# akio-tomiya/LatticeQCD.jl

Measured on AMD Instinct MI355X. Metric: CG iters/sec (D^+D) & Dslash GFLOP/s, 32^3x64 SU(3) Wilson fp64, higher is better.
Workload: dtype f64; 1 GPU; configs[3]: 32x32x32x64 Wilson D^+D CG (fixed-length window), fp64; dslash_variant=1, xcd_remap=2, xcd_nsub=16, xcd_ysplit=4, cg_fused=3, gauge_recon=12, gauge_recon_active=1, comm_backend=none, comm_requested=auto

## Files before the change

latticeqcd.jl_amd/csrc/capi.hip:

```cpp
#include "lqcd_internal.h"

#include <algorithm>
#include <cstdio>
#include <cstdlib>
#include <cstring>
#include <mutex>

namespace lqcd {

static thread_local std::string g_err;
static std::mutex g_live_mu;
static std::vector<const lqcd_ctx_s*> g_live;
bool ctx_is_live(const lqcd_ctx_s* c) {
    std::lock_guard<std::mutex> lk(g_live_mu);
    for (const lqcd_ctx_s* p : g_live)
        if (p == c) return true;
    return false;
}
static void ctx_set_live(const lqcd_ctx_s* c, bool live) {
    std::lock_guard<std::mutex> lk(g_live_mu);
    for (size_t i = 0; i < g_live.size(); i++)
        if (g_live[i] == c) { g_live.erase(g_live.begin() + i); break; }
    if (live) g_live.push_back(c);
}
// ... 283 lines not shown
    if (!strcmp(key, "clover_hop_s")) return &c->tun.clover_hop_s;
    if (!strcmp(key, "mixed_lean_residual")) return &c->tun.mixed_lean_residual;
    if (!strcmp(key, "mixed_xfuse")) return &c->tun.mixed_xfuse;
    if (!strcmp(key, "mixed_defer_x")) return &c->tun.mixed_defer_x;
    if (!strcmp(key, "pair32_active")) return &c->tun.pair32_active;
    if (!strcmp(key, "stag_both")) return &c->tun.stag_both;
    if (!strcmp(key, "clover_fused")) return &c->tun.clover_fused;
    if (!strcmp(key, "clover_transport")) return &c->tun.clover_transport;
    if (!strcmp(key, "halo_stream_mode")) return &c->tun.halo_stream_mode;
    if (!strcmp(key, "cg_skip_done")) return &c->tun.cg_skip_done;
    if (!strcmp(key, "cg_small")) return &c->tun.cg_small;
    if (!strcmp(key, "cg_tgauge")) return &c->tun.cg_tgauge;
    if (!strcmp(key, "tgauge_active")) return &c->tun.tgauge_active;
    if (!strcmp(key, "cg_sweep_alt")) return &c->tun.cg_sweep_alt;
    if (!strcmp(key, "cg_sweep_alt_active")) return &c->tun.cg_sweep_alt_active;
    if (!strcmp(key, "dslash_sweep")) return &c->tun.dslash_sweep;
    if (!strcmp(key, "sweep_rev_active")) return &c->tun.sweep_rev_active;
    if (!strcmp(key, "dslash_xshare")) return &c->tun.dslash_xshare;
    if (!strcmp(key, "xshare_active")) return &c->tun.xshare_active;
    if (!strcmp(key, "dslash_yshare")) return &c->tun.dslash_yshare;
    if (!strcmp(key, "yshare_active")) return &c->tun.yshare_active;
    if (!strcmp(key, "nt_centre")) return &c->tun.nt_centre;
    if (!strcmp(key, "cg_persist")) return &c->tun.cg_persist;
    if (!strcmp(key, "md_remap")) return &c->tun.md_remap;
    if (!strcmp(key, "staple_recon")) return &c->tun.staple_recon;
    if (!strcmp(key, "staple_tile")) return &c->tun.staple_tile;
    if (!strcmp(key, "md_reunitarize")) return &c->tun.md_reunitarize;
    if (!strcmp(key, "nt_blas")) return &c->tun.nt_blas;
    if (!strcmp(key, "cg_fold_scalars")) return &c->tun.cg_fold_scalars;
    if (!strcmp(key, "halo_fuse")) return &c->tun.halo_fuse;
// ... 45 lines not shown
extern "C" int lqcd_ctx_set_param(lqcd_ctx_t c, const char* key, int value) {
    ARGCHK(c && key, "lqcd_ctx_set_param: null");
    if (!strcmp(key, "adopt_thread")) {
        {
            std::lock_guard<std::mutex> lk(g_live_mu);
            c->home_thread = std::this_thread::get_id();
        }
        return ctx_drain_parked(c);
    }
    int* p = param_ptr(c, key);
    ARGCHK(p, std::string("lqcd_ctx_set_param: unknown key ") + key);
    if (!strcmp(key, "dslash_block")) ARGCHK(value == 64 || value == 128 || value == 256, "dslash_block must be 64, 128 or 256");
    if (!strcmp(key, "halo_stream_mode")) ARGCHK(value >= -1 && value <= 4, "halo_stream_mode must be -1 (timed once) or 0..4");
    if (!strcmp(key, "cg_rring")) ARGCHK(value == 0 || value == 2 || value == 4 || value == 8, "cg_rring must be 0 (off), 2, 4 or 8 (it divides the 8 iterations of a captured burst)");
    if (!strcmp(key, "cg_rring_mult")) ARGCHK((value == 1 || value == 2 || value == 4) && std::max(c->tun.cg_rring, 1) * value <= RRING_MAX, "cg_rring_mult must be 1, 2 or 4 with cg_rring x cg_rring_mult <= 32");
    if (!strcmp(key, "scratch_max")) ARGCHK(value >= 0, "scratch_max: 0 (no limit) or the number of work fields the scratch pool may hold");
    if (!strcmp(key, "bicg_fused")) ARGCHK(value != 3, "bicg_fused must be 0, 1, 2 or 4 (3, the grid-barrier form, was measured slower and removed)");
    if (!strcmp(key, "halo_inject_us")) ARGCHK(value >= 0 && value <= 100000, "halo_inject_us: 0..100000");
    if ((!strcmp(key, "lazy_links") || !strcmp(key, "lazy_merge")) && !value) LQCHK(links_flush_of(c));
    if (*p != value) LQCHK(links_flush_of(c));
    *p = value;
    if (!strcmp(key, "cg_rring_mult")) c->tun.cg_rring_mult_set = 1;
    return LQCD_OK;
}
extern "C" int lqcd_ctx_get_param(lqcd_ctx_t c, const char* key, int* value) {
    ARGCHK(c && key && value, "lqcd_ctx_get_param: null");
    if (!strcmp(key, "dw_active")) { *value = c->tun.dw_active; return LQCD_OK; }
    if (!strcmp(key, "adopt_thread")) {
        std::lock_guard<std::mutex> lk(g_live_mu);
        *value = std::this_thread::get_id() == c->home_thread ? 1 : 0;
        return LQCD_OK;
    }
    if (!strcmp(key, "parked_fields")) {
        std::lock_guard<std::mutex> lk(g_live_mu);
        *value = (int)c->parked_gauges.size();
        return LQCD_OK;
    }
// ... 100 lines not shown
```

latticeqcd.jl_amd/csrc/cg.hip:

```cpp
#include "ops_internal.h"
#include "stencil_common.h"

#include <algorithm>
#include <cmath>

namespace lqcd {


__global__ void cg_scalar_alpha(double* s) {
    if (s[S_DONE] != 0.0) { s[S_XDONE] = 1.0; return; }
    s[S_ALPHA] = s[S_RR] / s[S_PQ];
}
__global__ void cg_scalar_beta(double* s) {
    if (s[S_DONE] != 0.0) return;
    const double rrn = s[S_RRNEW];
    s[S_BETA] = rrn / s[S_RR];
    s[S_RR] = rrn;
    s[S_ITERS] += 1.0;
    if (rrn < s[S_EPS]) s[S_DONE] = 1.0;
}

__global__ __launch_bounds__(UB) void cg_update_xr(const double* __restrict__ s, double2* __restrict__ x, double2* __restrict__ r,
                                                    const double2* __restrict__ p, const double2* __restrict__ q, size_t n,
                                                    double* partial) {
// ... 441 lines not shown
    StencilCall s1;
    if (m == 0) {
        LQCHK(cg_batch_launch(c, x, w, 0));
        apply_bc(c, op->bc);
        LQCHK(make_full_call(op, w.tmp, w.p, 0, s1));
        s1.skip_flag = c->tun.cg_skip_done ? c->d_scal : nullptr;
    } else {
        apply_bc(c, op->bc);
        LQCHK(make_full_call(op, w.tmp, rk, 0, s1));
        s1.upd_scal = c->d_scal;
        s1.upd[0] = spinor_block(w.tmp, 0);
        s1.upd[1] = spinor_block(w.tmp, 1);
        s1.upd_rec = 1;
    }
    s1.gauge12t = gt;
    s1.norm_partial = c->d_partial;
    LQCHK(stencil_apply(c, s1));
    LQCHK(reduce_to_slot(c, nbs, 1, S_PQ, true, m == 0 ? 9 : 7));
    apply_bc(c, op->bc);
    StencilCall s2;
    LQCHK(make_full_call(op, rn, w.tmp, 1, s2));
    s2.gauge12t = gt;
    s2.sweep_rev = w.sweep_alt ? 1 : 0;
    s2.norm_partial = c->d_partial;
    s2.upd_scal = c->d_scal;
    for (int q = 0; q < 2; q++) { s2.upd[q] = spinor_block(rn, q); s2.upd_src[q] = spinor_block(rk, q); }
    LQCHK(stencil_apply(c, s2));
    LQCHK(reduce_to_slot(c, nbs, 1, S_RRNEW, true, 8));
    w.k++;
    return LQCD_OK;
}
static int cg_rring_wanted(lqcd_op_s* op, const CgWork& w) {
    lqcd_ctx_s* c = op->ctx;
    const int K = c->tun.cg_rring;
    if (c->tun.cg_fused < 3 || !(K == 2 || K == 4 || K == 8)) return 0;
    if (op->kind != LQCD_WILSON || op->r != 1.0 || op->csw != 0.0 || any_partitioned(c) || c->has_comm || !c->local_peers.empty()) return 0;
    if (!stencil_sdir_applies(c, op->kind, op->r, op_fused_clover(op))) return 0;
    StencilCall s;
// ... 77 lines not shown
    const int nbs = stencil_num_partials(c, op->kind, op->r, 2, 0, op_fused_clover(op));
    const bool defer = w.form == CgForm::DeferX;
    const bool ringed = defer && w.ring > 2;
    lqcd_spinor_s* pk = ringed ? w.buf(w.k % w.ring) : (defer && (w.k & 1)) ? w.q : w.p;
    lqcd_spinor_s* po = ringed ? w.buf((w.k + 1) % w.ring) : (defer && (w.k & 1)) ? w.p : w.q;
    const bool fold = c->has_comm && defer && c->tun.cg_fold_scalars;
    const bool part = any_partitioned(c) && c->has_comm && c->local_peers.empty();
    const bool folded = part && halo_fold_applies(c, op->kind, op->r, 2, 0, op_fused_clover(op));
    const bool fr = part && (c->tun.halo_fuse & 1) && !folded;
    const bool fp = part && defer && (c->tun.halo_fuse & 2) && op->kind == LQCD_WILSON && op->r == 1.0;
    {
        apply_bc(c, op->bc);
        StencilCall s1;
        LQCHK(make_full_call(op, w.tmp, pk, 0, s1));
        s1.gauge12t = gt;
        s1.norm_partial = c->d_partial;
        s1.skip_flag = c->tun.cg_skip_done ? c->d_scal : nullptr;
        if (fr) s1.red_slot = S_PQ;
        if (fp) { s1.pack_next = 1; s1.prepacked = (w.p_packed && w.pack_epoch == c->halo_epoch) ? 1 : 0; s1.defer_pack = folded ? 1 : 0; }
        LQCHK(stencil_apply(c, s1));
    }
    LQCHK(fr ? reduce_tail(c, 1, S_PQ, fold ? 0 : 1) : reduce_pack_to_slot(c, nbs, S_PQ, fold ? 0 : 1));
    apply_bc(c, op->bc);
    StencilCall s2;
    LQCHK(make_full_call(op, po, w.tmp, 1, s2));
    s2.gauge12t = gt;
    s2.sweep_rev = w.sweep_alt ? 1 : 0;
    s2.norm_partial = c->d_partial;
    if (fold) s2.scal_w = c->d_scal;
    s2.upd_scal = c->d_scal;
    s2.upd[0] = spinor_block(w.r, 0);
    s2.upd[1] = spinor_block(w.r, 1);
    if (fr) s2.red_slot = S_RRNEW;
    if (fp) s2.prepacked = 1;
    LQCHK(stencil_apply(c, s2));
    LQCHK(fr ? reduce_tail(c, 1, S_RRNEW, fold ? 0 : 2) : reduce_to_slot(c, nbs, 1, S_RRNEW, true, fold ? 0 : 2));
    const int nbu = stream_grid(c, n);
    HArgs h = HArgs();
    int npx = 0, npack = 0;
    if (fp) {
        int nt = 0;
        for (int mu = 0; mu < 4; mu++)
// ... 55 lines not shown
    if (!ok) for (lqcd_spinor_s*& f : w.more) { if (f) scratch_put(f); f = nullptr; }
    return ok;
}
static CgForm cg_choose_form(lqcd_op_s* op, CgWork& w) {
    lqcd_ctx_s* c = op->ctx;
    const int fused = c->tun.cg_fused;
    if (fused >= 2 && c->tun.cg_small && cg_small_ok(op, stencil_num_partials(c, op->kind, op->r, 2, 0, op_fused_clover(op)))) return CgForm::Small;
    if (const int K = cg_rring_wanted(op, w)) {
        for (int M = cg_rring_mult_wanted(op, K); M >= 1; M >>= 1)
            if (cg_more_get(c, w, K * M)) { w.rring = K * M; w.rring_k = K; return CgForm::RRing; }
    }
    if (fused >= 2 && c->tun.cg_defer_x) return CgForm::DeferX;
    return fused >= 2 ? CgForm::Fused : fused ? CgForm::NormFused : CgForm::Reference;
}

int cg_setup(lqcd_op_s* op, lqcd_spinor_s* x, lqcd_spinor_s* b, CgWork& w, double eps, double* rr0) {
    lqcd_ctx_s* c = op->ctx;
    const size_t n = x->elems;
    LQCHK(halo_schedule_settle(op));
    w.tgauge = cg_tgauge_wanted(op);
    c->tun.tgauge_active = w.tgauge ? 1 : 0;
    w.links_t = w.tgauge ? op->gauge->data12t : nullptr;
    w.gfix = w.tgauge ? op->gauge->gfix : nullptr;
    w.gauge_version = op->gauge->version;
    if (w.tgauge) LQCHK(spinor_gauge_rotate(c, w.gfix, x->data, x->data, 0));
    LQCHK(op_apply_async(op, w.tmp, x, 0, nullptr, nullptr, w.links_t));
    LQCHK(op_apply_async(op, w.q, w.tmp, 1, nullptr, nullptr, w.links_t));
    if (w.tgauge) LQCHK(spinor_gauge_rotate(c, w.gfix, w.r->data, b->data, 0));
    else HIPCHK(hipMemcpyAsync(w.r->data, b->data, n * sizeof(double2), hipMemcpyDeviceToDevice, c->stream));
    LQCHK(blas_axpy(c, -1.0, 0.0, w.q->data, w.r->data, n));
    HIPCHK(hipMemcpyAsync(w.p->data, w.r->data, n * sizeof(double2), hipMemcpyDeviceToDevice, c->stream));
    LQCHK(blas_norm2(c, w.r->data, n, rr0, true));
    double init[12] = {*rr0, 0, 0, 0, 0, 0, eps, 0, 0, 0, 0, 0};
    static_assert(S_BSTART - S_RR == 11, "cg_setup: the scalar block it initialises ends at S_BSTART");
    HIPCHK(hipMemcpyAsync(c->d_scal + S_RR, init, sizeof(init), hipMemcpyHostToDevice, c->stream));
    HIPCHK(hipStreamSynchronize(c->stream));
    w.k = 0; w.p_packed = false; w.flushed = false;
    w.rring = w.rring_k = 0;
    w.form = cg_choose_form(op, w);
    c->tun.cg_rring_active = w.rring_k;
    c->tun.cg_rring_depth_active = w.rring;
    w.sweep_alt = c->tun.cg_sweep_alt != 0 && w.tgauge && (w.form == CgForm::RRing || w.form == CgForm::Fused || w.form == CgForm::DeferX);
    c->tun.cg_sweep_alt_active = w.sweep_alt ? 1 : 0;
    w.ring = 2;
    if (w.form == CgForm::DeferX) {
        int want = cg_ring_wanted(op);
        if (c->tun.graph != 0 && !any_partitioned(c) && (8 % want) != 0) want = 2;
        if (cg_more_get(c, w, want)) w.ring = want;
    }
    return LQCD_OK;
}

int cg_run(lqcd_op_s* op, lqcd_spinor_s* x, lqcd_spinor_s* b, double eps, int maxiter, bool fixed, int* iters, double* final_rr) {
    lqcd_ctx_s* c = op->ctx;
    HIPCHK(hipSetDevice(c->device));
    CgWork w;
    int st = cg_work_get(c, x->kind, w);
    double rr = 0;
// ... 167 lines not shown
```

latticeqcd.jl_amd/csrc/lqcd_internal.h:

```cpp
#pragma once
#include <hip/hip_runtime.h>
#include <rccl/rccl.h>
#include <stdint.h>
#include <mutex>
#include <string>
#include <thread>
#include <vector>

#include "../../include/lqcd_hip.h"

namespace lqcd {

#ifdef LQCD_F32
typedef float real;
typedef float2 real2;
#define LQCD_PNS p32
inline namespace p32 {}
namespace p64 {}
#else
typedef double real;
typedef double2 real2;
#define LQCD_PNS p64
inline namespace p64 {}
namespace p32 {}
// ... 412 lines not shown
    int halo_fold_active = 0;
    int halo_fuse = 2;
    int cg_fold_scalars = 1;
    int nt_blas = 1;
    int md_reunitarize = 1;
    int staple_recon = 1;
    int staple_tile = 1;
    int md_remap = 1;
    int cg_defer_x = 1;
    int cg_persist = 1;
    int cg_small = 1;
    int cg_tgauge = 1;
    int tgauge_active = 0;
    int cg_sweep_alt = 1;
    int cg_sweep_alt_active = 0;
    int dslash_sweep = 0;
    int sweep_rev_active = 0;
    int dslash_xshare = 1;
    int xshare_active = 0;
    int dslash_yshare = 1;
    int yshare_active = 0;
    int nt_centre = 1;
    int cg_skip_done = 1;
    int clover_transport = 0;
    int stag_both = 0;
    int mixed_defer_x = 1;
    int mixed_xfuse = 0;
    int mixed_pair32 = 1;
    int mixed_action_solver = 0;
    int gauge_recon = 12;
// ... 366 lines not shown
    int kind;
    const double2* gauge;
    double2* out[2];
    const double2* in[2];
    const double2* xin[2];
    double a, b;
    double r;
    int dagger;
    int parity_mode;
    double* norm_partial = nullptr;
    const double* upd_scal = nullptr;
    double2* upd[2] = {nullptr, nullptr};
    const double2* upd_src[2] = {nullptr, nullptr};
    int upd_rec = 0;
    int sweep_rev = 0;
    const double* skip_flag = nullptr;
    const double* alpha_partials = nullptr;
    int alpha_n = 0;
    double* scal_w = nullptr;
    const double2* gauge12 = nullptr;
    const double2* gauge12t = nullptr;
    const void* gauge16 = nullptr;
    int gauge12_delta = 0;
    const double2* clover = nullptr;
    int prec = 0;
    int red_slot = -1;
    int pack_next = -1;
    double2* xacc[2] = {nullptr, nullptr};
    const double2* pacc[2] = {nullptr, nullptr};
    int prepacked = 0;
// ... 77 lines not shown
int clover_apply(lqcd_ctx_s* c, const double2* clov, lqcd_spinor_s* out, lqcd_spinor_s* in);
int clover_apply_parity(lqcd_ctx_s* c, const double2* clov, int parity, double2* out, const double2* in, double sa, const double2* z, double sz);
int clover_invert(lqcd_ctx_s* c, const double2* clov, double2* inv);
size_t clover_lambda_elems(const Geom& g);
int stout_gather_ext(lqcd_ctx_s* c, const lqcd_gauge_s* U, const double2* lamN, lqcd_gauge_s* G, double rho);
double2* stout_lambda_buffer(lqcd_ctx_s* c);
int clover_force(lqcd_ctx_s* c, const lqcd_gauge_s* U, lqcd_gauge_s* out, lqcd_spinor_s* X, lqcd_spinor_s* Y, double2* lam, double kappa,
                 double csw, double scale, int accumulate);

double2* spinor_block(lqcd_spinor_s* s, int p);
int gauge_ensure_recon12(lqcd_gauge_s* g);
int gauge_ensure_recon12d(lqcd_gauge_s* g);
int gauge_ensure_tgauge(lqcd_gauge_s* g);
int spinor_gauge_rotate(lqcd_ctx_s* c, const double2* gfix, double2* dst, const double2* src, int adjoint);
bool stencil_sdir_applies(lqcd_ctx_s* c, int kind, double r, bool clover);
bool stencil_tgauge_applies(lqcd_ctx_s* c, int kind, double r, bool clover);
int plaquette_local_sum(lqcd_gauge_s* g, const double2* const ghost[4], double* sum);
int gauge_pack_face(lqcd_gauge_s* g, int mu, double2* dst);

int links_flush(lqcd_ctx_s* c);
bool ctx_park_gauge(lqcd_gauge_s* g);
int ctx_drain_parked(lqcd_ctx_s* c);
int gauge_destroy_now(lqcd_gauge_s* g);
std::mutex& view_mutex();
bool ctx_is_live(const lqcd_ctx_s* c);
inline int links_flush_of(lqcd_ctx_s* c) { return (c && c->lazy.busy()) ? links_flush(c) : LQCD_OK; }
inline int links_flush_of(lqcd_gauge_s* g) { return g ? links_flush_of(g->ctx) : LQCD_OK; }
inline int links_flush_of(lqcd_op_s* o) { return o ? links_flush_of(o->ctx) : LQCD_OK; }

lqcd_spinor_s* scratch_get(lqcd_ctx_s* c, int kind, int subset);
// ... 4 lines not shown
```

latticeqcd.jl_amd/csrc/ops_internal.h:

```cpp
#pragma once
#include "lqcd_internal.h"

#include <functional>
#include <vector>

namespace lqcd {

double2* spinor_block(lqcd_spinor_s* s, int p);
int stream_grid(lqcd_ctx_s* c, size_t n);

StencilCall make_hop_call(lqcd_op_s* op, lqcd_spinor_s* out, lqcd_spinor_s* in, lqcd_spinor_s* xin, double a, double b, int dagger);
int check_full(lqcd_op_s* op, lqcd_spinor_s* a, lqcd_spinor_s* b, const char* who);
int make_full_call(lqcd_op_s* op, lqcd_spinor_s* out, lqcd_spinor_s* in, int dagger, StencilCall& s);
void apply_bc(lqcd_ctx_s* c, const int bc[4]);
void split_general_r(const StencilCall& s, StencilCall& s1, StencilCall& s2);

constexpr int UB = 256;
enum class CgForm { Unset, Reference, NormFused, Fused, DeferX, Small, RRing };
struct CgWork {
    lqcd_spinor_s *r, *p, *q, *tmp;
    uint64_t pack_epoch = 0;
    bool p_packed = false;
    CgForm form = CgForm::Unset;
    int k = 0;
    int ring = 2;
    lqcd_spinor_s* more[RRING_MAX - 2] = {};
    lqcd_spinor_s* buf(int j) const { return j == 0 ? p : j == 1 ? q : more[j - 2]; }
    int rring = 0;
    int rring_k = 0;
    bool flushed = false;
    lqcd_spinor_s* slot(int j) const { return j == 0 ? r : j == 1 ? q : more[j - 2]; }
    bool tgauge = false;
    const double2* links_t = nullptr;
    const double2* gfix = nullptr;
    uint64_t gauge_version = 0;
    bool sweep_alt = false;
};
int cg_work_get(lqcd_ctx_s* c, int kind, CgWork& w);
void cg_work_put(CgWork& w);
int cg_enqueue_iteration(lqcd_op_s* op, lqcd_spinor_s* x, CgWork& w);
int cg_flush_x(lqcd_op_s* op, lqcd_spinor_s* x, CgWork& w);
int cg_setup(lqcd_op_s* op, lqcd_spinor_s* x, lqcd_spinor_s* b, CgWork& w, double eps, double* rr0);
int cg_finish(lqcd_op_s* op, lqcd_spinor_s* x, CgWork& w, bool flush = true);
bool cg_gauge_moved(lqcd_op_s* op, const CgWork& w);
bool cg_persist_ok(lqcd_op_s* op);
int cg_persist_run(lqcd_op_s* op, lqcd_spinor_s* x, lqcd_spinor_s* b, CgWork& w, double eps, int maxiter, int* iters, double* rr, bool* converged, bool* gave_up);
typedef std::function<int(double2* out, const double2* in)> ApplyFn;
int cg_generic(lqcd_ctx_s* c, const ApplyFn& A, size_t n, double2* x, const double2* b, double2* r, double2* p, double2* q, double eps,
               int maxiter, int* iters, double* final_rr);
int cg_launch_update_xp(lqcd_ctx_s* c, double2* x, double2* p, const double2* r, size_t n);

// ... 112 lines not shown
```

latticeqcd.jl_amd/csrc/stencil.hip:

```cpp
#include "stencil_common.h"

#include <cstring>
namespace lqcd {
inline namespace LQCD_PNS {

template <int TB, bool DAG, bool RGEN>
__global__ __launch_bounds__(TB) void wilson_interior(KArgs k) {
    if (upd_done(k)) return;
    const real al_upd = update_alpha(k);
    int chunk, p;
    map_block(k, chunk, p);
    const int Vh = sp_stride(k.g);
    const int i = chunk * TB + threadIdx.x;
    const bool valid = i < k.g.Vh;
    real nrm = 0.0;
    if (valid) {
        Nbr n;
        int c[4];
        neighbours(k.g, p, i, n, c);
        cd acc[12], xv[12];
#pragma unroll
        for (int j = 0; j < 12; j++) acc[j] = mk(0.0, 0.0);
        if (k.a != 0.0) {
#pragma unroll
// ... 274 lines not shown
    real2* dst[2];
    const real2* usrc[2];
    int rec;
    const real2* in[2];
    const real2* xin[2];
    double* norm_partial;
    const double* upd_scal;
    const double* skip;
    double* scal_w;
    real a, b;
    int nt_store;
    int nt_centre;
    int xshare;
    int yshare;
    int sweep_rev, nslab;
    int nvirt, both, pmode;
    int XH, L1, L2, LT, nch;
    FastDiv dXH;
    real sgn_f[4], sgn_b[4];
    int cps, cpp, cpr, per_pass, ty, tz, ysplit;
    FastDiv d_perpass, d_cpr, d_ysplit, d_ty, d_cpp;
    unsigned* ctr;
    int per_wg;
    const real2* dotz[2];
    const real2* dotz2[2];
    double* dot_partial;
    int dot_conj;
    int ls;
    unsigned long long slice_bytes;
    FastDiv d_ls;
// ... 340 lines not shown
        u[j].re = face ? dg : u[j].re;
        u[j].im = face ? real(0.0) : u[j].im;
    }
}

__host__ __device__ constexpr bool sdir_xshare_instance(bool r12, bool delta) {
#if defined(LQCD_F32) || LQCD_SDIR_BOTH || LQCD_SDIR_GLDS
    return false;
#else
    return true;
#endif
}

__host__ __device__ constexpr bool sdir_yshare_instance(bool r12, bool delta) { return r12 && sdir_xshare_instance(r12, delta); }

template <int MU, bool DAG, bool R12, bool NTB, bool DOT = false, bool DELTA = false, bool DW5 = false, bool FOLD = false, bool CINV = false, bool TG = false>
__device__ inline void sdir_wave(const PipeArgs& a_, real2 (*part)[12][64], int lane, real al_upd, real& nrm, real& dre, real& dim, int vb, real& dre2, real& dim2) {
    int vblock = vb, s5 = 0;
    if constexpr (DW5) {
        const int g8 = (int)(blockIdx.x >> 3), gq = fdiv_nb(g8, a_.d_ls);
        s5 = g8 - gq * a_.ls;
        vblock = gq * 8 + (int)(blockIdx.x & 7);
    }
    PipeArgs a5;
    if constexpr (DW5) {
        a5 = a_;
        const unsigned long long off = (unsigned long long)s5 * a_.slice_bytes;
        a5.in[0] = boff64(a_.in[0], off); a5.in[1] = boff64(a_.in[1], off);
        a5.xin[0] = boff64(a_.xin[0], off); a5.xin[1] = boff64(a_.xin[1], off);
        a5.dst[0] = const_cast<real2*>(boff64(a_.dst[0], off)); a5.dst[1] = const_cast<real2*>(boff64(a_.dst[1], off));
    }
    const PipeArgs& a = DW5 ? a5 : a_;
// ... 2 lines not shown
    constexpr int FF = MU == 3 ? (SF > 0 ? 6 : 0) : 0;
    constexpr int FB = MU == 3 ? (SF > 0 ? 0 : 6) : 0;
    constexpr int NL = DELTA ? 8 : (R12 ? 6 : 9);
#ifdef LQCD_F32
    constexpr bool LATE_R = false;
#else
    constexpr bool LATE_R = DELTA || !R12;
#endif
    constexpr bool RING = !DOT && !DW5 && !FOLD && !CINV;
    constexpr bool XS = MU == 0 && RING && sdir_xshare_instance(R12, DELTA);
    const bool xs = XS && a_.xshare != 0;
    constexpr bool YSI = RING && sdir_yshare_instance(R12, DELTA);
    const bool ysh = YSI && a_.xshare != 0 && a_.yshare != 0;
    constexpr bool YS = MU == 1 && YSI;
    const bool ys = YS && ysh;
    const size_t gpar = (size_t)a.nch * 4 * NL * 64;
    const PipeSite s = pipe_site<MU, NL>(a, vblock, lane);
    cd xv[3] = {mk(0, 0), mk(0, 0), mk(0, 0)}, rv[3] = {mk(0, 0), mk(0, 0), mk(0, 0)};
    const bool z_is_x = DOT && (s.p ? a.dotz[1] == a.xin[1] : a.dotz[0] == a.xin[0]) && a.a != real(0.0);
    const bool two = DOT && z_is_x && (s.p ? a.dotz2[1] : a.dotz2[0]) != nullptr;
    auto load_z = [&]() {
        if (!z_is_x) {
#pragma unroll
            for (int cc = 0; cc < 3; cc++) rv[cc] = ld(boff(s.p ? a.dotz[1] : a.dotz[0], s.own) + co12(3 * MU + cc));
        } else if (two) {
#pragma unroll
            for (int cc = 0; cc < 3; cc++) rv[cc] = ld(boff(s.p ? a.dotz2[1] : a.dotz2[0], s.own) + co12(3 * MU + cc));
        }
    };
    if constexpr (DOT) {
// ... 307 lines not shown
                const cd dd = ld(ab + (size_t)(r >> 1) * 64);
                const real d = (r & 1) ? dd.im : dd.re;
                cd y = mk(d * chi[r].re, d * chi[r].im);
#pragma unroll
                for (int q = 0; q < 6; q++) {
                    if (q == r) continue;
                    const int lo = q < r ? q : r, hi = q < r ? r : q;
                    const cd m = ld(ab + (size_t)(3 + 5 * lo - (lo * (lo - 1)) / 2 + (hi - lo - 1)) * 64);
                    if (q > r) cfma(y, m, chi[q]); else cfma_conj(y, m, chi[q]);
                }
                hs[cc] = mk(hs[cc].re + wgt * y.re, hs[cc].im + wgt * y.im);
            }
            __builtin_amdgcn_sched_barrier(0);
        }
    }
#pragma unroll
    for (int cc = 0; cc < 3; cc++) {
        const int j = 3 * MU + cc;
        const real2 s0 = part[0][j][lane], s1 = part[1][j][lane], s2 = part[2][j][lane], s3 = part[3][j][lane];
        cd sm = CINV ? hs[cc] : mk((s0.x + s1.x) + (s2.x + s3.x), (s0.y + s1.y) + (s2.y + s3.y));
        cd v = a.b * sm;
        v = mk(fma(a.a, xv[cc].re, v.re), fma(a.a, xv[cc].im, v.im));
        if constexpr (DW5) v = mk(v.re + w5[cc].re, v.im + w5[cc].im);
        if constexpr (DOT) {
            const cd z = z_is_x ? xv[cc] : rv[cc];
            nrm = fma(v.re, v.re, nrm); nrm = fma(v.im, v.im, nrm);
            if (a.nt_store) st_nt(dstp + co12(j), v); else st(dstp + co12(j), v);
            dre = fma(z.re, v.re, dre); dre = fma(z.im, v.im, dre);
            dim = fma(z.re, v.im, dim); dim = fma(-z.im, v.re, dim);
            if (two) {
                const cd z2 = rv[cc];
                dre2 = fma(z2.re, v.re, dre2); dre2 = fma(z2.im, v.im, dre2);
                dim2 = fma(z2.re, v.im, dim2); dim2 = fma(-z2.im, v.re, dim2);
            }
        } else if (a.upd_scal) {
            cd r = rv[cc];
            if (RING && a.rec) {
                r.re = fma(al_upd, r.re, v.re); r.im = fma(al_upd, r.im, v.im);
                nrm = fma(r.re, r.re, nrm); nrm = fma(r.im, r.im, nrm);
                if (a.nt_store) st_nt(dstp + co12(j), r); else st(dstp + co12(j), r);
            } else {
                r.re = fma(-al_upd, v.re, r.re); r.im = fma(-al_upd, v.im, r.im);
                nrm = fma(r.re, r.re, nrm); nrm = fma(r.im, r.im, nrm);
                st(dstp + co12(j), r);
            }
        } else {
            nrm = fma(v.re, v.re, nrm); nrm = fma(v.im, v.im, nrm);
            if (a.nt_store) st_nt(dstp + co12(j), v); else st(dstp + co12(j), v);
        }
    }
}

template <bool DAG, bool R12, bool NTB, bool DOT, bool DELTA, bool DW5, bool FOLD, bool CINV, bool TG>
__device__ __forceinline__ void dirsplit_s_block(const PipeArgs& a, real2 (*part)[12][64], double* red) {
    if ((a.upd_scal && a.upd_scal[S_DONE] != 0.0) || (a.skip && a.skip[S_DONE] != 0.0)) {
        if (a.scal_w && blockIdx.x == 0 && threadIdx.x == 0) a.scal_w[S_XDONE] = 1.0;
        return;
    }
    real al_upd = real(0);
    if (a.upd_scal) {
        if (!DOT && !DW5 && !FOLD && !CINV && a.rec) al_upd = (real)a.upd_scal[S_BETA];
        else if (a.scal_w) {
            const double rr = a.upd_scal[S_RR];
// ... 2 lines not shown
            al_upd = (real)al;
        } else al_upd = (real)a.upd_scal[S_ALPHA];
    }
    int vb = (int)blockIdx.x;
    if constexpr (FOLD) {
        if (a.vlist) vb = a.vlist[blockIdx.x];
        if (a.fsel) {
            int p_, t, z, yc;
            pipe_map(a, vb, p_, t, z, yc);
            const int y0 = fdiv(yc * 64, a.dXH), y1 = fdiv(yc * 64 + 63, a.dXH);
            const bool bnd = (((a.fold >> 3) & 1) && (t == 0 || t == a.LT - 1)) || (((a.fold >> 2) & 1) && (z == 0 || z == a.L2 - 1)) ||
                             (((a.fold >> 1) & 1) && (y0 == 0 || y1 == a.L1 - 1));
            if ((a.fsel == 1) == bnd) return;
        }
    }
    if constexpr (!DOT && !DELTA && !DW5 && !FOLD && !CINV) {
        if (a.sweep_rev) {
            int j = vb >> 3;
            const int pb = a.both ? (j & 1) : 0;
            j = a.both ? (j >> 1) : j;
            const int q = fdiv_nb(j, a.d_cpr);
            j += (a.nslab - 1 - 2 * q) * a.cpr;
            vb = ((a.both ? 2 * j + pb : j) << 3) | (vb & 7);
        }
    }
    const int w = __builtin_amdgcn_readfirstlane(threadIdx.x >> 6);
    const int lane = threadIdx.x & 63;
    real nrm = 0.0, dre = 0.0, dim = 0.0, dre2 = 0.0, dim2 = 0.0;
    switch (w) {
    case 0: sdir_wave<0, DAG, R12, NTB, DOT, DELTA, DW5, FOLD, CINV, TG>(a, part, lane, al_upd, nrm, dre, dim, vb, dre2, dim2); break;
    case 1: sdir_wave<1, DAG, R12, NTB, DOT, DELTA, DW5, FOLD, CINV, TG>(a, part, lane, al_upd, nrm, dre, dim, vb, dre2, dim2); break;
    case 2: sdir_wave<2, DAG, R12, NTB, DOT, DELTA, DW5, FOLD, CINV, TG>(a, part, lane, al_upd, nrm, dre, dim, vb, dre2, dim2); break;
    default: sdir_wave<3, DAG, R12, NTB, DOT, DELTA, DW5, FOLD, CINV, TG>(a, part, lane, al_upd, nrm, dre, dim, vb, dre2, dim2); break;
    }
    if constexpr (DOT) {
        const bool five = a.dotz2[0] != nullptr || a.dotz2[1] != nullptr;
        double t3[5] = {(double)dre, (double)((a.dot_conj & 1) ? -dim : dim), (double)nrm, (double)dre2, (double)dim2};
#pragma unroll
        for (int q = 0; q < 5; q++) {
            if (q < 3 || five) {
                t3[q] = wave_sum(t3[q]);
                if (lane == 0) red[4 * q + w] = t3[q];
            }
        }
        __syncthreads();
        const int nv = five ? 5 : 3;
        if ((int)threadIdx.x < nv) a.dot_partial[(a.dot_conj & 2) ? (size_t)threadIdx.x * gridDim.x + blockIdx.x : nv * (size_t)blockIdx.x + threadIdx.x] =
            (red[4 * threadIdx.x] + red[4 * threadIdx.x + 1]) + (red[4 * threadIdx.x + 2] + red[4 * threadIdx.x + 3]);
// ... 598 lines not shown

static PipeArgs make_pipe_args(lqcd_ctx_s* c, const KArgs& k, const StencilCall& s) {
    PipeArgs a;
    a.gauge = k.gauge12 ? k.gauge12 : k.gauge;
    const bool upd = k.upd_scal != nullptr;
    for (int p = 0; p < 2; p++) { a.usrc[p] = s.upd_src[p] ? (const real2*)s.upd_src[p] : k.upd[p]; }
    a.rec = s.upd_rec;
    for (int p = 0; p < 2; p++) { a.dst[p] = upd ? k.upd[p] : k.out[p]; a.in[p] = k.in[p]; a.xin[p] = k.xin[p]; a.dotz[p] = k.dotz[p]; a.dotz2[p] = k.dotz2[p]; }
    a.dot_partial = k.dot_partial; a.dot_conj = k.dot_conj;
    a.clover = k.clover;
    a.norm_partial = k.norm_partial; a.upd_scal = k.upd_scal; a.skip = k.skip; a.scal_w = k.scal_w;
    a.a = k.a; a.b = k.b;
    a.nt_store = (k.nt & 4) != 0;
    a.nt_centre = c->tun.nt_centre != 0;
    a.xshare = 0; a.yshare = 0;
    a.sweep_rev = 0; a.nslab = 0;
    a.nvirt = k.nblocks; a.both = s.parity_mode == 2; a.pmode = s.parity_mode == 2 ? 0 : s.parity_mode;
    a.XH = k.g.XH; a.L1 = k.g.L[1]; a.L2 = k.g.L[2]; a.LT = k.g.L[3]; a.nch = k.g.nch; a.dXH = k.g.dXH;
    for (int mu = 0; mu < 4; mu++) {
        a.sgn_f[mu] = k.g.part[mu] ? real(0.0) : real(k.g.bc_fwd[mu]);
        a.sgn_b[mu] = k.g.part[mu] ? real(0.0) : real(k.g.bc_bwd[mu]);
    }
    a.cps = k.cps; a.cpp = k.cpp; a.cpr = k.cpr; a.per_pass = std::max(1, k.cpr * k.g.L[3]); a.ty = k.ty; a.tz = k.tz; a.ysplit = k.ysplit;
    a.ctr = c->pipe_ctr; a.per_wg = 1;
    a.d_perpass = k.d_perpass; a.d_cpr = k.d_cpr; a.d_ysplit = k.d_ysplit; a.d_ty = k.d_ty; a.d_cpp = make_fastdiv(std::max(1, k.cpp));
    a.ls = s.dw_ls; a.slice_bytes = (unsigned long long)s.dw_slice * sizeof(real2); a.d_ls = make_fastdiv(std::max(1, s.dw_ls)); a.dw_mass = (real)s.dw_mass;
    a.fold = 0;
    a.fsel = s.fold >= 2 ? s.fold - 1 : 0;
    a.vlist = nullptr;
    for (int mu = 0; mu < 4; mu++) {
        const size_t cnt = (size_t)(s.parity_mode == 2 ? 2 : 1) * 6 * face_half_sites(c->geom, mu);
        a.gh_b[mu] = (const real2*)halo_recv_base(c, mu); a.gh_f[mu] = (const real2*)halo_recv_base(c, mu) + cnt;
        a.Fh[mu] = face_half_sites(c->geom, mu);
        a.gsf[mu] = (c->coord[mu] == c->pe[mu] - 1) ? real(c->geom.bc_fwd[mu]) : real(1.0);
        a.gsb[mu] = (c->coord[mu] == 0) ? real(c->geom.bc_bwd[mu]) : real(1.0);
        if (s.fold && k.g.part[mu]) a.fold |= 1 << mu;
    }
    return a;
}

static void pipe_sweep_args(lqcd_ctx_s* c, const KArgs& k, const StencilCall& s, bool delta, PipeArgs& a) {
    const int par = s.parity_mode == 2 ? 2 : 1;
    const bool plain = c->tun.dslash_pipe == 2 && s.dw_ls <= 1 && !s.fold && !delta;
    const bool map_ok = k.cps > 0 && k.cpr > 0 && k.nblocks % (8 * par * k.cpr) == 0 && k.nblocks / (8 * par * k.cpr) == (k.nsub / 8) * k.g.L[3];
    a.nslab = map_ok ? k.nblocks / (8 * par * k.cpr) : 0;
    a.sweep_rev = 0;
    if (!plain || !map_ok) return;
    a.sweep_rev = s.sweep_rev ? 1 : 0;
    c->tun.sweep_rev_active = a.sweep_rev;
}

static void pipe_xshare_args(lqcd_ctx_s* c, const KArgs& k, const StencilCall& s, bool delta, PipeArgs& a) {
    a.xshare = 0; a.yshare = 0;
    if (kF32Build || c->tun.dslash_pipe != 2 || s.dw_ls > 1 || s.fold) return;
    const bool inst = sdir_xshare_instance(k.gauge12 != nullptr, delta);
    a.xshare = (inst && c->tun.dslash_xshare && k.g.XH == 16 && !k.g.part[0]) ? 1 : 0;
    c->tun.xshare_active = a.xshare;
    a.yshare = (a.xshare && sdir_yshare_instance(k.gauge12 != nullptr, delta) && c->tun.dslash_yshare && k.g.L[1] % 4 == 0 && !k.g.part[1]) ? 1 : 0;
    c->tun.yshare_active = a.yshare;
}

static HArgs make_hargs(lqcd_ctx_s* c, const StencilCall& s);

__global__ void fold_classify_s(PipeArgs a, int n, unsigned char* bnd) {
// ... 365 lines not shown
bool wilson_pipe_applies(lqcd_ctx_s* c, int kind, double r, int parity_mode, bool clover) {
    if (c->tun.dslash_variant != 1 || !c->tun.dslash_pipe || clover || kind != LQCD_WILSON || !use_dirsplit(c, kind, r)) return false;
    if (r != 1.0) return false;
    const Geom& g = c->geom;
    const int plane = g.XH * g.L[1];
    if (plane % 64 != 0 || c->tun.xcd_remap != 2 || (size_t)g.nch * 64 * 2304 >= ((size_t)1 << 32)) return false;
    if ((plane * g.L[2] / 64) % 8 != 0) return false;
    const int nvirt = ((g.Vh + 63) / 64) * (parity_mode == 2 ? 2 : 1);
    if (c->tun.dslash_pipe == 2 || c->tun.dslash_pipe == 3) return true;
    return nvirt >= std::max(1, c->tun.pipe_min_chunks) * wilson_pipe_grid(c, nvirt, 0);
}
bool stencil_sdir_applies(lqcd_ctx_s* c, int kind, double r, bool clover) {
    if (any_partitioned(c) || c->has_comm || c->tun.dslash_pipe != 2 || !(c->tun.gauge_recon == 12 || c->tun.dslash_s18)) return false;
    return wilson_pipe_applies(c, kind, r, 2, clover);
}
bool stencil_tgauge_applies(lqcd_ctx_s* c, int kind, double r, bool clover) {
    if (any_partitioned(c) || c->tun.dslash_pipe != 2 || c->tun.gauge_recon != 12 || c->geom.L[3] < 2) return false;
    return wilson_pipe_applies(c, kind, r, 2, clover);
}
bool halo_fold_applies(lqcd_ctx_s* c, int kind, double r, int parity_mode, int prec, bool clover) {
    if (!c->tun.halo_fold) return false;
    if (!any_partitioned(c) || !c->has_comm || !c->local_peers.empty()) return false;
    if ((kind != LQCD_WILSON && kind != LQCD_STAGGERED) || (prec != 0 && prec != 1)) return false;
    if (c->tun.dslash_variant != 1 || (c->tun.dslash_pipe != 0 && c->tun.dslash_pipe != 2)) return false;
    (void)r; (void)parity_mode; (void)clover;
    return true;
}
int stencil_num_partials(lqcd_ctx_s* c, int kind, double r, int parity_mode, int prec, bool clover) {
    const int nt = halo_fold_applies(c, kind, r, parity_mode, prec, clover) ? 0 : max_face_threads(c, parity_mode);
    return stencil_num_blocks(c, kind, r, parity_mode, prec, clover) + (nt > 0 ? ((nt + 127) / 128) * 8 : 0);
// ... 5 lines not shown
```

Measured before the change: 1260 iter/s.

## Store last slabs of CG stencil output with plain stores to keep them in cache

```diff
diff --git a/latticeqcd.jl_amd/csrc/capi.hip b/latticeqcd.jl_amd/csrc/capi.hip
--- a/latticeqcd.jl_amd/csrc/capi.hip
+++ b/latticeqcd.jl_amd/csrc/capi.hip
@@ -321,6 +321,8 @@
     if (!strcmp(key, "tgauge_active")) return &c->tun.tgauge_active;
     if (!strcmp(key, "cg_sweep_alt")) return &c->tun.cg_sweep_alt;
     if (!strcmp(key, "cg_sweep_alt_active")) return &c->tun.cg_sweep_alt_active;
+    if (!strcmp(key, "cg_store_keep_mb")) return &c->tun.cg_store_keep_mb;
+    if (!strcmp(key, "cg_store_keep_active")) return &c->tun.cg_store_keep_active;
     if (!strcmp(key, "dslash_sweep")) return &c->tun.dslash_sweep;
     if (!strcmp(key, "sweep_rev_active")) return &c->tun.sweep_rev_active;
     if (!strcmp(key, "dslash_xshare")) return &c->tun.dslash_xshare;
@@ -396,6 +398,7 @@
     if (!strcmp(key, "halo_stream_mode")) ARGCHK(value >= -1 && value <= 4, "halo_stream_mode must be -1 (timed once) or 0..4");
     if (!strcmp(key, "cg_rring")) ARGCHK(value == 0 || value == 2 || value == 4 || value == 8, "cg_rring must be 0 (off), 2, 4 or 8 (it divides the 8 iterations of a captured burst)");
     if (!strcmp(key, "cg_rring_mult")) ARGCHK((value == 1 || value == 2 || value == 4) && std::max(c->tun.cg_rring, 1) * value <= RRING_MAX, "cg_rring_mult must be 1, 2 or 4 with cg_rring x cg_rring_mult <= 32");
+    if (!strcmp(key, "cg_store_keep_mb")) ARGCHK(value >= -1, "cg_store_keep_mb: -1 (off), 0 (every store streams) or the MB of traffic at the end of a launch that store plain");
     if (!strcmp(key, "scratch_max")) ARGCHK(value >= 0, "scratch_max: 0 (no limit) or the number of work fields the scratch pool may hold");
     if (!strcmp(key, "bicg_fused")) ARGCHK(value != 3, "bicg_fused must be 0, 1, 2 or 4 (3, the grid-barrier form, was measured slower and removed)");
     if (!strcmp(key, "halo_inject_us")) ARGCHK(value >= 0 && value <= 100000, "halo_inject_us: 0..100000");
@@ -403,6 +406,7 @@
     if (*p != value) LQCHK(links_flush_of(c));
     *p = value;
     if (!strcmp(key, "cg_rring_mult")) c->tun.cg_rring_mult_set = 1;
+    if (!strcmp(key, "cg_store_keep_mb")) c->tun.cg_store_keep_mb_set = 1;
     return LQCD_OK;
 }
 extern "C" int lqcd_ctx_get_param(lqcd_ctx_t c, const char* key, int* value) {
diff --git a/latticeqcd.jl_amd/csrc/cg.hip b/latticeqcd.jl_amd/csrc/cg.hip
--- a/latticeqcd.jl_amd/csrc/cg.hip
+++ b/latticeqcd.jl_amd/csrc/cg.hip
@@ -479,6 +479,7 @@
         s1.upd_rec = 1;
     }
     s1.gauge12t = gt;
+    s1.keep_slabs = w.store_keep;
     s1.norm_partial = c->d_partial;
     LQCHK(stencil_apply(c, s1));
     LQCHK(reduce_to_slot(c, nbs, 1, S_PQ, true, m == 0 ? 9 : 7));
@@ -487,6 +488,7 @@
     LQCHK(make_full_call(op, rn, w.tmp, 1, s2));
     s2.gauge12t = gt;
     s2.sweep_rev = w.sweep_alt ? 1 : 0;
+    s2.keep_slabs = w.store_keep;
     s2.norm_partial = c->d_partial;
     s2.upd_scal = c->d_scal;
     for (int q = 0; q < 2; q++) { s2.upd[q] = spinor_block(rn, q); s2.upd_src[q] = spinor_block(rk, q); }
@@ -594,6 +596,7 @@
         StencilCall s1;
         LQCHK(make_full_call(op, w.tmp, pk, 0, s1));
         s1.gauge12t = gt;
+        s1.keep_slabs = w.store_keep;
         s1.norm_partial = c->d_partial;
         s1.skip_flag = c->tun.cg_skip_done ? c->d_scal : nullptr;
         if (fr) s1.red_slot = S_PQ;
@@ -606,6 +609,7 @@
     LQCHK(make_full_call(op, po, w.tmp, 1, s2));
     s2.gauge12t = gt;
     s2.sweep_rev = w.sweep_alt ? 1 : 0;
+    s2.keep_slabs = w.store_keep;
     s2.norm_partial = c->d_partial;
     if (fold) s2.scal_w = c->d_scal;
     s2.upd_scal = c->d_scal;
@@ -691,6 +695,7 @@
     return fused >= 2 ? CgForm::Fused : fused ? CgForm::NormFused : CgForm::Reference;
 }
 
+constexpr int CG_STENCIL_BYTES = 864;
 int cg_setup(lqcd_op_s* op, lqcd_spinor_s* x, lqcd_spinor_s* b, CgWork& w, double eps, double* rr0) {
     lqcd_ctx_s* c = op->ctx;
     const size_t n = x->elems;
@@ -719,6 +724,16 @@
     c->tun.cg_rring_depth_active = w.rring;
     w.sweep_alt = c->tun.cg_sweep_alt != 0 && w.tgauge && (w.form == CgForm::RRing || w.form == CgForm::Fused || w.form == CgForm::DeferX);
     c->tun.cg_sweep_alt_active = w.sweep_alt ? 1 : 0;
+    w.store_keep = -1;
+    if (w.sweep_alt && c->tun.cg_store_keep_mb >= 0 &&
+        (c->tun.cg_store_keep_mb_set || stencil_num_partials(c, op->kind, op->r, 2, 0, op_fused_clover(op)) > 1024)) {
+        const int nslab = stencil_sweep_slabs(c);
+        if (nslab > 0) {
+            const size_t slab_bytes = (size_t)CG_STENCIL_BYTES * (2 * (size_t)c->geom.Vh / nslab);
+            w.store_keep = (int)std::min<size_t>(((size_t)c->tun.cg_store_keep_mb << 20) / slab_bytes, (size_t)nslab);
+        }
+    }
+    c->tun.cg_store_keep_active = w.store_keep;
     w.ring = 2;
     if (w.form == CgForm::DeferX) {
         int want = cg_ring_wanted(op);
diff --git a/latticeqcd.jl_amd/csrc/lqcd_internal.h b/latticeqcd.jl_amd/csrc/lqcd_internal.h
--- a/latticeqcd.jl_amd/csrc/lqcd_internal.h
+++ b/latticeqcd.jl_amd/csrc/lqcd_internal.h
@@ -450,6 +450,9 @@
     int tgauge_active = 0;
     int cg_sweep_alt = 1;
     int cg_sweep_alt_active = 0;
+    int cg_store_keep_mb = 256;
+    int cg_store_keep_mb_set = 0;
+    int cg_store_keep_active = -1;
     int dslash_sweep = 0;
     int sweep_rev_active = 0;
     int dslash_xshare = 1;
@@ -846,6 +849,7 @@
     const double2* upd_src[2] = {nullptr, nullptr};
     int upd_rec = 0;
     int sweep_rev = 0;
+    int keep_slabs = -1;
     const double* skip_flag = nullptr;
     const double* alpha_partials = nullptr;
     int alpha_n = 0;
@@ -953,6 +957,7 @@
 int gauge_ensure_tgauge(lqcd_gauge_s* g);
 int spinor_gauge_rotate(lqcd_ctx_s* c, const double2* gfix, double2* dst, const double2* src, int adjoint);
 bool stencil_sdir_applies(lqcd_ctx_s* c, int kind, double r, bool clover);
+int stencil_sweep_slabs(lqcd_ctx_s* c);
 bool stencil_tgauge_applies(lqcd_ctx_s* c, int kind, double r, bool clover);
 int plaquette_local_sum(lqcd_gauge_s* g, const double2* const ghost[4], double* sum);
 int gauge_pack_face(lqcd_gauge_s* g, int mu, double2* dst);
diff --git a/latticeqcd.jl_amd/csrc/ops_internal.h b/latticeqcd.jl_amd/csrc/ops_internal.h
--- a/latticeqcd.jl_amd/csrc/ops_internal.h
+++ b/latticeqcd.jl_amd/csrc/ops_internal.h
@@ -35,6 +35,7 @@
     const double2* gfix = nullptr;
     uint64_t gauge_version = 0;
     bool sweep_alt = false;
+    int store_keep = -1;
 };
 int cg_work_get(lqcd_ctx_s* c, int kind, CgWork& w);
 void cg_work_put(CgWork& w);
diff --git a/latticeqcd.jl_amd/csrc/stencil.hip b/latticeqcd.jl_amd/csrc/stencil.hip
--- a/latticeqcd.jl_amd/csrc/stencil.hip
+++ b/latticeqcd.jl_amd/csrc/stencil.hip
@@ -312,6 +312,7 @@
     int xshare;
     int yshare;
     int sweep_rev, nslab;
+    int keep_from;
     int nvirt, both, pmode;
     int XH, L1, L2, LT, nch;
     FastDiv dXH;
@@ -682,8 +683,10 @@
 
 __host__ __device__ constexpr bool sdir_yshare_instance(bool r12, bool delta) { return r12 && sdir_xshare_instance(r12, delta); }
 
+__host__ __device__ constexpr bool sdir_keep_instance(bool r12, bool delta) { return r12 && !delta; }
+
 template <int MU, bool DAG, bool R12, bool NTB, bool DOT = false, bool DELTA = false, bool DW5 = false, bool FOLD = false, bool CINV = false, bool TG = false>
-__device__ inline void sdir_wave(const PipeArgs& a_, real2 (*part)[12][64], int lane, real al_upd, real& nrm, real& dre, real& dim, int vb, real& dre2, real& dim2) {
+__device__ inline void sdir_wave(const PipeArgs& a_, real2 (*part)[12][64], int lane, real al_upd, real& nrm, real& dre, real& dim, int vb, real& dre2, real& dim2, int keep = -1) {
     int vblock = vb, s5 = 0;
     if constexpr (DW5) {
         const int g8 = (int)(blockIdx.x >> 3), gq = fdiv_nb(g8, a_.d_ls);
@@ -716,6 +719,7 @@
     const bool ysh = YSI && a_.xshare != 0 && a_.yshare != 0;
     constexpr bool YS = MU == 1 && YSI;
     const bool ys = YS && ysh;
+    constexpr bool KEEP = RING && sdir_keep_instance(R12, DELTA);
     const size_t gpar = (size_t)a.nch * 4 * NL * 64;
     const PipeSite s = pipe_site<MU, NL>(a, vblock, lane);
     cd xv[3] = {mk(0, 0), mk(0, 0), mk(0, 0)}, rv[3] = {mk(0, 0), mk(0, 0), mk(0, 0)};
@@ -1053,6 +1057,7 @@
             __builtin_amdgcn_sched_barrier(0);
         }
     }
+    cd ov[KEEP ? 3 : 1];
 #pragma unroll
     for (int cc = 0; cc < 3; cc++) {
         const int j = 3 * MU + cc;
@@ -1077,15 +1082,29 @@
             if (RING && a.rec) {
                 r.re = fma(al_upd, r.re, v.re); r.im = fma(al_upd, r.im, v.im);
                 nrm = fma(r.re, r.re, nrm); nrm = fma(r.im, r.im, nrm);
-                if (a.nt_store) st_nt(dstp + co12(j), r); else st(dstp + co12(j), r);
+                if constexpr (KEEP) ov[cc] = r;
+                else { if (a.nt_store) st_nt(dstp + co12(j), r); else st(dstp + co12(j), r); }
             } else {
                 r.re = fma(-al_upd, v.re, r.re); r.im = fma(-al_upd, v.im, r.im);
                 nrm = fma(r.re, r.re, nrm); nrm = fma(r.im, r.im, nrm);
-                st(dstp + co12(j), r);
+                if constexpr (KEEP) ov[cc] = r;
+                else st(dstp + co12(j), r);
             }
         } else {
             nrm = fma(v.re, v.re, nrm); nrm = fma(v.im, v.im, nrm);
-            if (a.nt_store) st_nt(dstp + co12(j), v); else st(dstp + co12(j), v);
+            if constexpr (KEEP) ov[cc] = v;
+            else { if (a.nt_store) st_nt(dstp + co12(j), v); else st(dstp + co12(j), v); }
+        }
+    }
+    if constexpr (KEEP) {
+        const bool updm = a.upd_scal != nullptr && !a.rec;
+        const bool nt_out = keep < 0 ? (a.nt_store && !updm) : (keep == 0 && (a.nt_store || updm));
+        if (nt_out) {
+#pragma unroll
+            for (int cc = 0; cc < 3; cc++) st_nt(dstp + co12(3 * MU + cc), ov[cc]);
+        } else {
+#pragma unroll
+            for (int cc = 0; cc < 3; cc++) st(dstp + co12(3 * MU + cc), ov[cc]);
         }
     }
 }
@@ -1118,24 +1137,29 @@
             if ((a.fsel == 1) == bnd) return;
         }
     }
+    int keep = -1;
     if constexpr (!DOT && !DELTA && !DW5 && !FOLD && !CINV) {
-        if (a.sweep_rev) {
+        constexpr bool KI = sdir_keep_instance(R12, DELTA);
+        if (a.sweep_rev || (KI && a.keep_from >= 0)) {
             int j = vb >> 3;
             const int pb = a.both ? (j & 1) : 0;
             j = a.both ? (j >> 1) : j;
             const int q = fdiv_nb(j, a.d_cpr);
-            j += (a.nslab - 1 - 2 * q) * a.cpr;
-            vb = ((a.both ? 2 * j + pb : j) << 3) | (vb & 7);
+            if (KI && a.keep_from >= 0) keep = q >= a.keep_from ? 1 : 0;
+            if (a.sweep_rev) {
+                j += (a.nslab - 1 - 2 * q) * a.cpr;
+                vb = ((a.both ? 2 * j + pb : j) << 3) | (vb & 7);
+            }
         }
     }
     const int w = __builtin_amdgcn_readfirstlane(threadIdx.x >> 6);
     const int lane = threadIdx.x & 63;
     real nrm = 0.0, dre = 0.0, dim = 0.0, dre2 = 0.0, dim2 = 0.0;
     switch (w) {
-    case 0: sdir_wave<0, DAG, R12, NTB, DOT, DELTA, DW5, FOLD, CINV, TG>(a, part, lane, al_upd, nrm, dre, dim, vb, dre2, dim2); break;
-    case 1: sdir_wave<1, DAG, R12, NTB, DOT, DELTA, DW5, FOLD, CINV, TG>(a, part, lane, al_upd, nrm, dre, dim, vb, dre2, dim2); break;
-    case 2: sdir_wave<2, DAG, R12, NTB, DOT, DELTA, DW5, FOLD, CINV, TG>(a, part, lane, al_upd, nrm, dre, dim, vb, dre2, dim2); break;
-    default: sdir_wave<3, DAG, R12, NTB, DOT, DELTA, DW5, FOLD, CINV, TG>(a, part, lane, al_upd, nrm, dre, dim, vb, dre2, dim2); break;
+    case 0: sdir_wave<0, DAG, R12, NTB, DOT, DELTA, DW5, FOLD, CINV, TG>(a, part, lane, al_upd, nrm, dre, dim, vb, dre2, dim2, keep); break;
+    case 1: sdir_wave<1, DAG, R12, NTB, DOT, DELTA, DW5, FOLD, CINV, TG>(a, part, lane, al_upd, nrm, dre, dim, vb, dre2, dim2, keep); break;
+    case 2: sdir_wave<2, DAG, R12, NTB, DOT, DELTA, DW5, FOLD, CINV, TG>(a, part, lane, al_upd, nrm, dre, dim, vb, dre2, dim2, keep); break;
+    default: sdir_wave<3, DAG, R12, NTB, DOT, DELTA, DW5, FOLD, CINV, TG>(a, part, lane, al_upd, nrm, dre, dim, vb, dre2, dim2, keep); break;
     }
     if constexpr (DOT) {
         const bool five = a.dotz2[0] != nullptr || a.dotz2[1] != nullptr;
@@ -1764,7 +1788,7 @@
     a.nt_store = (k.nt & 4) != 0;
     a.nt_centre = c->tun.nt_centre != 0;
     a.xshare = 0; a.yshare = 0;
-    a.sweep_rev = 0; a.nslab = 0;
+    a.sweep_rev = 0; a.nslab = 0; a.keep_from = -1;
     a.nvirt = k.nblocks; a.both = s.parity_mode == 2; a.pmode = s.parity_mode == 2 ? 0 : s.parity_mode;
     a.XH = k.g.XH; a.L1 = k.g.L[1]; a.L2 = k.g.L[2]; a.LT = k.g.L[3]; a.nch = k.g.nch; a.dXH = k.g.dXH;
     for (int mu = 0; mu < 4; mu++) {
@@ -1789,15 +1813,19 @@
     return a;
 }
 
+static int pipe_nslab(const KArgs& k, int par) {
+    const bool map_ok = k.cps > 0 && k.cpr > 0 && k.nblocks % (8 * par * k.cpr) == 0 && k.nblocks / (8 * par * k.cpr) == (k.nsub / 8) * k.g.L[3];
+    return map_ok ? k.nblocks / (8 * par * k.cpr) : 0;
+}
 static void pipe_sweep_args(lqcd_ctx_s* c, const KArgs& k, const StencilCall& s, bool delta, PipeArgs& a) {
     const int par = s.parity_mode == 2 ? 2 : 1;
     const bool plain = c->tun.dslash_pipe == 2 && s.dw_ls <= 1 && !s.fold && !delta;
-    const bool map_ok = k.cps > 0 && k.cpr > 0 && k.nblocks % (8 * par * k.cpr) == 0 && k.nblocks / (8 * par * k.cpr) == (k.nsub / 8) * k.g.L[3];
-    a.nslab = map_ok ? k.nblocks / (8 * par * k.cpr) : 0;
-    a.sweep_rev = 0;
-    if (!plain || !map_ok) return;
+    a.nslab = pipe_nslab(k, par);
+    a.sweep_rev = 0; a.keep_from = -1;
+    if (!plain || a.nslab == 0) return;
     a.sweep_rev = s.sweep_rev ? 1 : 0;
     c->tun.sweep_rev_active = a.sweep_rev;
+    if (s.keep_slabs >= 0 && sdir_keep_instance(k.gauge12 != nullptr, delta)) a.keep_from = a.nslab - std::min(s.keep_slabs, a.nslab);
 }
 
 static void pipe_xshare_args(lqcd_ctx_s* c, const KArgs& k, const StencilCall& s, bool delta, PipeArgs& a) {
@@ -2193,6 +2221,12 @@
     if (any_partitioned(c) || c->has_comm || c->tun.dslash_pipe != 2 || !(c->tun.gauge_recon == 12 || c->tun.dslash_s18)) return false;
     return wilson_pipe_applies(c, kind, r, 2, clover);
 }
+int stencil_sweep_slabs(lqcd_ctx_s* c) {
+    if (c->tun.dslash_pipe != 2) return 0;
+    StencilCall s = StencilCall();
+    s.parity_mode = 2;
+    return pipe_nslab(make_kargs(c, s, 64), 2);
+}
 bool stencil_tgauge_applies(lqcd_ctx_s* c, int kind, double r, bool clover) {
     if (any_partitioned(c) || c->tun.dslash_pipe != 2 || c->tun.gauge_recon != 12 || c->geom.L[3] < 2) return false;
     return wilson_pipe_applies(c, kind, r, 2, clover);
```

Measured after the change: 1280 iter/s (median of 6 runs). 1.02x the previous value.
